# sdfgeoff/stereo_depth_estimation

Measured on AMD Instinct MI355X. Metric: stereo pairs/s training @320x240 bf16, 1/2/4/8 MI355X; EPE vs ref, higher is better.
Workload: dtype bf16

## Files before the change

stereo_depth_estimation_amd/csrc/bwd_fused.hip:

```cpp
#include <stdio.h>

#include "halo_util.h"

namespace {

typedef float f32x16 __attribute__((ext_vector_type(16)));

constexpr int FB_TH = 8, FB_TW = 16;
constexpr int FB_HW = FB_TW + 2, FB_HH = FB_TH + 2;
constexpr int FB_HPX = FB_HW * FB_HH;
constexpr int FB_NI = (FB_HPX * 4 + 255) / 256;
constexpr int FB_HSL = (FB_NI * 256 / 32) * 8;
static_assert(FB_TH * FB_TW == 128 && FB_TW % 16 == 0, "4 MFMA waves x 32 pixels; tr_pair rows p, p + 8 in one row");
constexpr int FB_DL = 40;
constexpr int FB_XL = 48;
constexpr int FB_XC = 64;
__device__ __forceinline__ int fb_xoff(int c) { return (c & 15) + (c >> 4) * FB_XC; }
constexpr int FB_WL = 9 * 32 + 8;
constexpr int FB_SL = 40;
constexpr int FB_DYH = FB_HSL * FB_DL, FB_XH = FB_HSL * FB_XL + (FB_XC - FB_XL + 16), FB_ST = FB_TH * FB_TW * FB_SL;
constexpr int FB_BUF = FB_DYH + FB_XH + FB_ST;
constexpr int FB_BLOCKS = 256;
#ifndef FB_EXP
#define FB_EXP 0
#endif
constexpr bool FB_DG = (FB_EXP & 32) != 0;
__device__ __forceinline__ unsigned long long fb_clk() {
    asm volatile("s_waitcnt lgkmcnt(0)" ::: "memory");
    return __builtin_amdgcn_s_memtime();
}

struct BwdArgs {
    const __bf16 *da, *y, *yp;
    const float *sc, *sh, *mu, *is, *coef;
    const float *psc, *psh, *pmu, *pis;
    const __bf16* wd;
    int kpad;
    int B, H, W, tiles_x, tiles_y;
    __bf16* dx;
    float* slab;
    float2* part;
    unsigned long long* dbg;
};

template <bool B> struct BoolC { static constexpr bool v = B; };

template <int PPX>
__device__ __forceinline__ int fb_pixel(int item) { return (item / (8 * PPX)) * 8 + (item & 7); }
template <int PPX>
__device__ __forceinline__ int fb_piece(int item) { return (item >> 3) % PPX; }

__device__ __forceinline__ void fb_tile(int tiles_x, int tiles_y, int bid, int nblk, int k, int& tx, int& ty, int& b) {
    const int strip = bid + (k / tiles_y) * nblk;
    ty = k % tiles_y;
    tx = strip % tiles_x;
    b = strip / tiles_x;
}
__device__ __forceinline__ int fb_ntile(int tiles_x, int tiles_y, int B, int bid, int nblk) {
    const int nstrips = tiles_x * B;
    return bid < nstrips ? ((nstrips - 1 - bid) / nblk + 1) * tiles_y : 0;
}

__global__ __launch_bounds__(512) void k_bwd_fused32(const BwdArgs p) {
    __shared__ __attribute__((aligned(16))) __bf16 smem[2 * FB_BUF];
    __shared__ __attribute__((aligned(16))) __bf16 wds[32 * FB_WL];
    __shared__ __attribute__((aligned(16))) __bf16 scr[4 * 32 * 32];
    __shared__ __attribute__((aligned(16))) float redf[4 * 32 * 2];

    const int tid = threadIdx.x, lane = tid & 63;
    const bool is_loader = tid >= 256;
    const int wid = (tid >> 6) & 3;
    const int bid = (blockIdx.x & 7) * (gridDim.x >> 3) + (blockIdx.x >> 3);
    const int t_begin = 0;
    const int ntile = fb_ntile(p.tiles_x, p.tiles_y, p.B, bid, gridDim.x);
    const int hw = p.H * p.W;

    for (int i = tid; i < 32 * 36; i += 512) {
        const int r = i / 36, c8 = i - r * 36;
        *reinterpret_cast<uint4*>(wds + r * FB_WL + c8 * 8) =
            *reinterpret_cast<const uint4*>(p.wd + (size_t)r * p.kpad + c8 * 8);
    }

    if (is_loader) {
        const int ltid = tid - 256;
        if (FB_EXP & 128) __builtin_amdgcn_s_setprio(1);
        const int piece = fb_piece<4>(ltid);
        constexpr unsigned OOB = 0x80000000u;
        float ksc[8], ksh[8], kB[8], kC[8];
#pragma unroll
        for (int j = 0; j < 8; ++j) {
            const int c = piece * 8 + j;
            const float k1 = p.coef[3 * c + 1], k2 = p.coef[3 * c + 2], is = p.is[c], sc = p.sc[c], sh = p.sh[c];
            ksc[j] = sc;
            ksh[j] = sh;
            kB[j] = -is * k2;
            kC[j] = is * k2 * sh + sc * (p.mu[c] * is * k2 - k1);
        }
        const float4 s0 = *reinterpret_cast<const float4*>(p.psc + piece * 8);
        const float4 s1 = *reinterpret_cast<const float4*>(p.psc + piece * 8 + 4);
        const float4 t0 = *reinterpret_cast<const float4*>(p.psh + piece * 8);
        const float4 t1 = *reinterpret_cast<const float4*>(p.psh + piece * 8 + 4);
        unsigned geo[FB_NI];
        int stash[FB_NI];
#pragma unroll
        for (int i = 0; i < FB_NI; ++i) {
            const int px = fb_pixel<4>(ltid + 256 * i);
            const int hy = px / FB_HW, hx = px - hy * FB_HW;
            geo[i] = px < FB_HPX ? (unsigned)(hy << 8 | hx) : 0xffffffffu;
            const bool in = px < FB_HPX && hy >= 1 && hy <= FB_TH && hx >= 1 && hx <= FB_TW;
            stash[i] = in ? ((hy - 1) * FB_TW + hx - 1) * FB_SL + piece * 8 : -1;
        }
        const bool w3 = (ltid & ~63) + 256 * (FB_NI - 1) < FB_HPX * 4;
        unsigned need = 0;
#pragma unroll
        for (int i = 0; i < FB_NI; ++i) need |= (unsigned)(geo[i] != 0xffffffffu) << i;
        struct Set {
            uint4 a[FB_NI], y[FB_NI], x[FB_NI];
            unsigned m;
            bool edge;
        };
        Set sa, sb;
        auto load = [&](Set& q, int tile) __attribute__((always_inline)) {
            if ((FB_EXP & 16) && tile >= t_begin + 2) return;
            const bool live = tile < t_begin + ntile;
            const int tl = live ? tile : t_begin;
            int tx, ty, b;
            fb_tile(p.tiles_x, p.tiles_y, bid, gridDim.x, tl, tx, ty, b);
            const int h0 = ty * FB_TH - 1, w0 = tx * FB_TW - 1;
            const size_t img = (size_t)b * hw * 32;
            const __amdgpu_buffer_rsrc_t ra =
                __builtin_amdgcn_make_buffer_rsrc((void*)(p.da + img), (short)0, hw * 64, 0x00020000);
            const __amdgpu_buffer_rsrc_t ry =
                __builtin_amdgcn_make_buffer_rsrc((void*)(p.y + img), (short)0, hw * 64, 0x00020000);
            const __amdgpu_buffer_rsrc_t rp =
                __builtin_amdgcn_make_buffer_rsrc((void*)(p.yp + img), (short)0, hw * 64, 0x00020000);
            unsigned m = 0;
#pragma unroll
            for (int i = 0; i < FB_NI; ++i) {
                if (i == FB_NI - 1 && !w3) break;
                const int h = h0 + (int)(geo[i] >> 8), w = w0 + (int)(geo[i] & 0xffu);
                const bool ok = live & (geo[i] != 0xffffffffu) & (h >= 0) & (h < p.H) & (w >= 0) & (w < p.W);
                m |= (unsigned)ok << i;
                const unsigned off = ok ? (unsigned)(h * p.W + w) * 64u + (unsigned)piece * 16u : OOB;
                const auto va = __builtin_amdgcn_raw_buffer_load_b128(ra, off, 0, 0);
                const auto vy = __builtin_amdgcn_raw_buffer_load_b128(ry, off, 0, 0);
                const auto vp = __builtin_amdgcn_raw_buffer_load_b128(rp, off, 0, 0);
                q.a[i] = make_uint4(va[0], va[1], va[2], va[3]);
                q.y[i] = make_uint4(vy[0], vy[1], vy[2], vy[3]);
                q.x[i] = make_uint4(vp[0], vp[1], vp[2], vp[3]);
            }
            q.m = m;
            q.edge = __builtin_amdgcn_ballot_w64(m != (w3 ? need : need & ((1u << (FB_NI - 1)) - 1))) != 0;
        };
        auto store = [&](Set& q, int buf) __attribute__((always_inline)) {
            __bf16* dyh = smem + buf * FB_BUF;
            __bf16* xh = dyh + FB_DYH;
            __bf16* st = xh + FB_XH;
            auto put = [&](auto SEL) __attribute__((always_inline)) {
#pragma unroll
                for (int i = 0; i < FB_NI; ++i) {
                    if (i == FB_NI - 1 && !w3) break;
                    const bool ok = (q.m >> i) & 1u;
                    const int px = fb_pixel<4>(ltid + 256 * i);
                    uint4 d = (FB_EXP & 1) ? q.a[i] : bn_bwd_pk(q.a[i], q.y[i], ksc, ksh, kB, kC);
                    uint4 x = (FB_EXP & 1) ? q.x[i] : bnrelu_pk(q.x[i], s0, s1, t0, t1);
                    if constexpr (decltype(SEL)::v) {
                        d = ok ? d : make_uint4(0, 0, 0, 0);
                        x = ok ? x : make_uint4(0, 0, 0, 0);
                    }
                    *reinterpret_cast<uint4*>(dyh + px * FB_DL + piece * 8) = d;
                    *reinterpret_cast<uint4*>(xh + px * FB_XL + fb_xoff(piece * 8)) = x;
                    if (stash[i] >= 0) *reinterpret_cast<uint4*>(st + stash[i]) = q.x[i];
                }
            };
            if (q.edge)
                put(BoolC<true>{});
            else
                put(BoolC<false>{});
        };
        load(sa, t_begin);
        __builtin_amdgcn_sched_barrier(0);
        load(sb, t_begin + 1);
        __syncthreads();
        unsigned long long tc[5] = {0, 0, 0, 0, 0}, tm0 = 0, t_all = FB_DG ? fb_clk() : 0;
        auto stamp = [&](int k) __attribute__((always_inline)) {
            if (FB_DG) {
                const unsigned long long t1 = fb_clk();
                tc[k] += t1 - tm0;
                tm0 = t1;
            }
        };
        for (int i = 0; i < ntile; i += 2) {
            if (FB_DG) {
                tm0 = fb_clk();
                asm volatile("s_waitcnt vmcnt(9)" ::: "memory");
                stamp(3);
            }
            store(sa, 0);
            stamp(0);
            load(sa, t_begin + i + 2);
            stamp(1);
            __syncthreads();
            stamp(2);
            if (FB_DG) {
                asm volatile("s_waitcnt vmcnt(9)" ::: "memory");
                stamp(3);
            }
            store(sb, 1);
            stamp(0);
            load(sb, t_begin + i + 3);
            stamp(1);
            __syncthreads();
            stamp(2);
        }
        if (FB_DG && p.dbg && lane == 0) {
            unsigned long long* d = p.dbg + ((size_t)bid * 8 + 4 + wid) * 8;
            d[0] = tc[0];
            d[1] = tc[1];
            d[2] = tc[2];
            d[3] = tc[3];
            d[4] = fb_clk() - t_all;
            d[5] = ntile;
        }
        __syncthreads();
        return;
    }

    __syncthreads();
    const int g = lane >> 4, q4 = (lane & 15) >> 2, pp = lane & 3;
    const int pk = 4 * (g >> 1) + q4, ch16 = 16 * (g & 1) + 4 * pp;
    const int tw0 = wid, tw1 = wid + 4;
    const int toffx0 = ((tw0 / 3) * FB_HW + tw0 % 3) * FB_XL, toffx1 = ((tw1 / 3) * FB_HW + tw1 % 3) * FB_XL;
    f32x16 accw[3];
#pragma unroll
    for (int t = 0; t < 3; ++t)
#pragma unroll
        for (int r = 0; r < 16; ++r) accw[t][r] = 0.f;
    BnsK bk[4];
    {
        const int c = (lane & 3) * 8;
#pragma unroll
        for (int q = 0; q < 4; ++q) {
            float v[4][2];
#pragma unroll
            for (int h = 0; h < 2; ++h) {
                const int ch = c + 2 * q + h;
                v[0][h] = p.psc[ch];
                v[1][h] = p.psh[ch];
                v[2][h] = p.pis[ch];
                v[3][h] = -p.pmu[ch] * p.pis[ch];
            }
            bk[q].sc = f32x2{v[0][0], v[0][1]};
            bk[q].sh = f32x2{v[1][0], v[1][1]};
            bk[q].is = f32x2{v[2][0], v[2][1]};
            bk[q].nmi = f32x2{v[3][0], v[3][1]};
        }
    }
    float own[16];
#pragma unroll
    for (int j = 0; j < 16; ++j) own[j] = 0.f;
    __bf16* const scw = scr + wid * 32 * 32;
    auto swz = [](int j, int px) { return j ^ ((px >> 1) & 3); };
    unsigned long long tc[6] = {0, 0, 0, 0, 0, 0}, t0 = 0, t_all = FB_DG ? fb_clk() : 0;
    auto stamp = [&](int k) __attribute__((always_inline)) {
        if (FB_DG) {
            const unsigned long long t1 = fb_clk();
            tc[k] += t1 - t0;
            t0 = t1;
        }
    };
    auto epilogue = [&](const f32x16& acc, const uint4* yv, int tl) __attribute__((always_inline)) {
        uint2 pk2[4];
#pragma unroll
        for (int g4 = 0; g4 < 4; ++g4) {
            bf16x4 v;
#pragma unroll
            for (int q = 0; q < 4; ++q) v[q] = (__bf16)acc[4 * g4 + q];
            pk2[g4] = *reinterpret_cast<uint2*>(&v);
        }
#pragma unroll
        for (int k = 0; k < 4; k += 2) {
            const auto rx = __builtin_amdgcn_permlane32_swap(pk2[k].x, pk2[k + 1].x, false, false);
            const auto ry = __builtin_amdgcn_permlane32_swap(pk2[k].y, pk2[k + 1].y, false, false);
            const int px = lane & 31, j = k + (lane >> 5);
            *reinterpret_cast<uint4*>(scw + px * 32 + swz(j, px) * 8) = make_uint4(rx[0], ry[0], rx[1], ry[1]);
        }
        asm volatile("" ::: "memory");
        int tx, ty, b;
        fb_tile(p.tiles_x, p.tiles_y, bid, gridDim.x, tl, tx, ty, b);
        const __amdgpu_buffer_rsrc_t rd = __builtin_amdgcn_make_buffer_rsrc(
            (void*)(p.dx + (size_t)b * hw * 32), (short)0, hw * 64, 0x00020000);
        uint4 vv[2];
#pragma unroll
        for (int rr = 0; rr < 2; ++rr) {
            const int px = rr * 16 + (lane >> 2), j = lane & 3;
            vv[rr] = *reinterpret_cast<const uint4*>(scw + px * 32 + swz(j, px) * 8);
        }
        asm volatile("" ::: "memory");
#pragma unroll
        for (int rr = 0; rr < 2; ++rr) {
            const int q = wid * 32 + rr * 16 + (lane >> 2), j = lane & 3;
            const int h = ty * FB_TH + q / FB_TW, w = tx * FB_TW + q % FB_TW;
            bns_add(own, vv[rr], yv[rr], true, bk);
            __attribute__((ext_vector_type(4))) unsigned data = {vv[rr].x, vv[rr].y, vv[rr].z, vv[rr].w};
            __builtin_amdgcn_raw_buffer_store_b128(data, rd, (unsigned)(h * p.W + w) * 64u + (unsigned)j * 16u, 0, 2);
        }
    };
    f32x16 accp;
    uint4 yvp[2];
    auto tile = [&](int it, auto EPI) __attribute__((always_inline)) {
        if (FB_DG) t0 = fb_clk();
        __syncthreads();
        stamp(0);
        const __bf16* dyh = smem + (it & 1) * FB_BUF;
        const __bf16* xh = dyh + FB_DYH;
        const __bf16* st = xh + FB_XH;
#pragma unroll
        for (int rr = 0; rr < FB_TH; ++rr) {
            const int r = (2 * wid + rr) & (FB_TH - 1);
            const __bf16* a0 = dyh + ((r + 1) * FB_HW + 1 + pk) * FB_DL + ch16;
            const bf16x8 af = tr_pair(a0, a0 + 8 * FB_DL);
            const __bf16* xr = xh + (r * FB_HW + pk) * FB_XL + fb_xoff(ch16);
            const bf16x8 b0 = tr_pair(xr + toffx0, xr + toffx0 + 8 * FB_XL);
            const bf16x8 b1 = tr_pair(xr + toffx1, xr + toffx1 + 8 * FB_XL);
            accw[0] = __builtin_amdgcn_mfma_f32_32x32x16_bf16(af, b0, accw[0], 0, 0, 0);
            accw[1] = __builtin_amdgcn_mfma_f32_32x32x16_bf16(af, b1, accw[1], 0, 0, 0);
            if (rr < 2) {
                const __bf16* x8 = xr + (2 * FB_HW + 2) * FB_XL;
                accw[2] = __builtin_amdgcn_mfma_f32_32x32x16_bf16(af, tr_pair(x8, x8 + 8 * FB_XL), accw[2], 0, 0, 0);
            }
            if constexpr (decltype(EPI)::v)
                if (rr == 2) epilogue(accp, yvp, t_begin + it - 1);
        }
        stamp(1);
        f32x16 accd;
#pragma unroll
        for (int r = 0; r < 16; ++r) accd[r] = 0.f;
        const int c8 = 8 * (lane >> 5);
        const __bf16* wrow = wds + (lane & 31) * FB_WL + c8;
        const int qd = wid * 32 + (lane & 31);
        const __bf16* drow = dyh + ((qd / FB_TW) * FB_HW + qd % FB_TW) * FB_DL + c8;
#pragma unroll
        for (int tap = 0; tap < 9; ++tap) {
            const int toff = ((tap / 3) * FB_HW + tap % 3) * FB_DL;
#pragma unroll
            for (int kk = 0; kk < 2; ++kk) {
                const bf16x8 a = *reinterpret_cast<const bf16x8*>(wrow + tap * 32 + kk * 16);
                const bf16x8 b = *reinterpret_cast<const bf16x8*>(drow + toff + kk * 16);
                accd = __builtin_amdgcn_mfma_f32_32x32x16_bf16(a, b, accd, 0, 0, 0);
            }
        }
        accp = accd;
#pragma unroll
        for (int rr = 0; rr < 2; ++rr) {
            const int px = rr * 16 + (lane >> 2), j = lane & 3;
            yvp[rr] = *reinterpret_cast<const uint4*>(st + (wid * 32 + px) * FB_SL + j * 8);
        }
        stamp(2);
    };
    if (ntile > 0) tile(0, BoolC<false>{});
    for (int it = 1; it < ntile; ++it) tile(it, BoolC<true>{});
    if (ntile > 0) epilogue(accp, yvp, t_begin + ntile - 1);
    if (FB_DG && p.dbg && lane == 0) {
        unsigned long long* d = p.dbg + ((size_t)bid * 8 + wid) * 8;
#pragma unroll
        for (int k = 0; k < 6; ++k) d[k] = tc[k];
        d[6] = fb_clk() - t_all;
        d[7] = ntile;
    }
    if (ntile & 1) __syncthreads();

    float* slab = p.slab + (size_t)bid * 32 * 288;
    float* red8 = reinterpret_cast<float*>(smem + (ntile & 1) * FB_BUF);
    static_assert(FB_BUF * 2 >= 4 * 1024 * 4, "tap-8 partials fit one halo buffer");
#pragma unroll
    for (int i = 0; i < 16; ++i) {
        const int co = 8 * (i / 4) + 4 * (lane >> 5) + i % 4, ci = lane & 31;
        slab[(size_t)co * 288 + tw0 * 32 + ci] = accw[0][i];
        slab[(size_t)co * 288 + tw1 * 32 + ci] = accw[1][i];
        red8[wid * 1024 + co * 32 + ci] = accw[2][i];
    }
#pragma unroll
    for (int k = 0; k < 16; ++k)
#pragma unroll
        for (int o = 4; o < 64; o <<= 1) own[k] += __shfl_xor(own[k], o);
    if (lane < 4) {
#pragma unroll
        for (int k = 0; k < 16; ++k)
            redf[(wid * 32 + lane * 8 + k / 2) * 2 + (k & 1)] = own[(k & ~3) | ((k & 1) << 1) | ((k >> 1) & 1)];
    }
    __syncthreads();
#pragma unroll
    for (int e = tid; e < 1024; e += 256)
        slab[(size_t)(e >> 5) * 288 + 8 * 32 + (e & 31)] = (red8[e] + red8[1024 + e]) + (red8[2048 + e] + red8[3072 + e]);
    if (tid < 32) {
        float s = 0.f, sx = 0.f;
#pragma unroll
        for (int w = 0; w < 4; ++w) {
            s += redf[(w * 32 + tid) * 2];
            sx += redf[(w * 32 + tid) * 2 + 1];
        }
        p.part[(size_t)bid * 32 + tid] = make_float2(s, sx);
    }
}


struct DecArgs {
    const __bf16 *da, *y, *xu, *xs;
    const float *sc, *sh, *mu, *is, *coef;
    const float *ssc, *ssh;
    const __bf16* wd;
    int kpad;
    int B, H, W, tiles_x, tiles_y;
    __bf16 *du, *dsk;
    float* slab;
    float2* part;
    unsigned long long* dbg;
};
constexpr int FD_BUF = FB_DYH + 2 * FB_XH;

__global__ __launch_bounds__(512) void k_bwd_fused_dec(const DecArgs p) {
    __shared__ __attribute__((aligned(16))) __bf16 smem[2 * FD_BUF];
    __shared__ __attribute__((aligned(16))) __bf16 wds[64 * FB_WL];
    __shared__ __attribute__((aligned(16))) __bf16 scr[4 * 32 * 32];
    __shared__ __attribute__((aligned(16))) float redf[4 * 32];

    const int tid = threadIdx.x, lane = tid & 63;
    const bool is_loader = tid >= 256;
    const int wid = (tid >> 6) & 3;
    const int bid = (blockIdx.x & 7) * (gridDim.x >> 3) + (blockIdx.x >> 3);
    const int t_begin = 0;
    const int ntile = fb_ntile(p.tiles_x, p.tiles_y, p.B, bid, gridDim.x);
    const int hw = p.H * p.W;
    auto tile_of = [&](int tl, int& tx, int& ty, int& b) __attribute__((always_inline)) {
        fb_tile(p.tiles_x, p.tiles_y, bid, gridDim.x, tl, tx, ty, b);
    };

    for (int i = tid; i < 64 * 36; i += 512) {
        const int r = i / 36, c8 = i - r * 36;
        *reinterpret_cast<uint4*>(wds + r * FB_WL + c8 * 8) =
            *reinterpret_cast<const uint4*>(p.wd + (size_t)r * p.kpad + c8 * 8);
    }

    if (is_loader) {
        const int ltid = tid - 256;
        const int piece = fb_piece<4>(ltid);
        constexpr unsigned OOB = 0x80000000u;
        float ksc[8], ksh[8], kB[8], kC[8];
#pragma unroll
        for (int j = 0; j < 8; ++j) {
            const int c = piece * 8 + j;
            const float k1 = p.coef[3 * c + 1], k2 = p.coef[3 * c + 2], is = p.is[c], sc = p.sc[c], sh = p.sh[c];
            ksc[j] = sc;
            ksh[j] = sh;
            kB[j] = -is * k2;
            kC[j] = is * k2 * sh + sc * (p.mu[c] * is * k2 - k1);
        }
        const float4 s0 = *reinterpret_cast<const float4*>(p.ssc + piece * 8);
        const float4 s1 = *reinterpret_cast<const float4*>(p.ssc + piece * 8 + 4);
        const float4 t0 = *reinterpret_cast<const float4*>(p.ssh + piece * 8);
        const float4 t1 = *reinterpret_cast<const float4*>(p.ssh + piece * 8 + 4);
        unsigned geo[FB_NI];
#pragma unroll
        for (int i = 0; i < FB_NI; ++i) {
            const int px = fb_pixel<4>(ltid + 256 * i);
            const int hy = px / FB_HW, hx = px - hy * FB_HW;
            geo[i] = px < FB_HPX ? (unsigned)(hy << 8 | hx) : 0xffffffffu;
        }
        const bool w3 = (ltid & ~63) + 256 * (FB_NI - 1) < FB_HPX * 4;
        unsigned need = 0;
#pragma unroll
        for (int i = 0; i < FB_NI; ++i) need |= (unsigned)(geo[i] != 0xffffffffu) << i;
        struct Set {
            uint4 a[FB_NI], y[FB_NI], u[FB_NI], s[FB_NI];
            unsigned m;
            bool edge;
        };
        Set sa, sb;
        auto load = [&](Set& q, int tile) __attribute__((always_inline)) {
            const bool live = tile < t_begin + ntile;
            int tx, ty, b;
            tile_of(live ? tile : t_begin, tx, ty, b);
            const int h0 = ty * FB_TH - 1, w0 = tx * FB_TW - 1;
            const size_t img = (size_t)b * hw * 32;
            const __amdgpu_buffer_rsrc_t ra =
                __builtin_amdgcn_make_buffer_rsrc((void*)(p.da + img), (short)0, hw * 64, 0x00020000);
            const __amdgpu_buffer_rsrc_t ry =
                __builtin_amdgcn_make_buffer_rsrc((void*)(p.y + img), (short)0, hw * 64, 0x00020000);
            const __amdgpu_buffer_rsrc_t ru =
                __builtin_amdgcn_make_buffer_rsrc((void*)(p.xu + img), (short)0, hw * 64, 0x00020000);
            const __amdgpu_buffer_rsrc_t rs =
                __builtin_amdgcn_make_buffer_rsrc((void*)(p.xs + img), (short)0, hw * 64, 0x00020000);
            unsigned m = 0;
#pragma unroll
            for (int i = 0; i < FB_NI; ++i) {
                if (i == FB_NI - 1 && !w3) break;
                const int h = h0 + (int)(geo[i] >> 8), w = w0 + (int)(geo[i] & 0xffu);
                const bool ok = live & (geo[i] != 0xffffffffu) & (h >= 0) & (h < p.H) & (w >= 0) & (w < p.W);
                m |= (unsigned)ok << i;
                const unsigned off = ok ? (unsigned)(h * p.W + w) * 64u + (unsigned)piece * 16u : OOB;
                const auto va = __builtin_amdgcn_raw_buffer_load_b128(ra, off, 0, 0);
                const auto vy = __builtin_amdgcn_raw_buffer_load_b128(ry, off, 0, 0);
                const auto vu = __builtin_amdgcn_raw_buffer_load_b128(ru, off, 0, 0);
                const auto vs = __builtin_amdgcn_raw_buffer_load_b128(rs, off, 0, 0);
                q.a[i] = make_uint4(va[0], va[1], va[2], va[3]);
                q.y[i] = make_uint4(vy[0], vy[1], vy[2], vy[3]);
                q.u[i] = make_uint4(vu[0], vu[1], vu[2], vu[3]);
                q.s[i] = make_uint4(vs[0], vs[1], vs[2], vs[3]);
            }
            q.m = m;
            q.edge = __builtin_amdgcn_ballot_w64(m != (w3 ? need : need & ((1u << (FB_NI - 1)) - 1))) != 0;
        };
        auto store = [&](Set& q, int buf) __attribute__((always_inline)) {
            __bf16* dyh = smem + buf * FD_BUF;
            __bf16* xuh = dyh + FB_DYH;
            __bf16* xsh = xuh + FB_XH;
            auto put = [&](auto SEL) __attribute__((always_inline)) {
#pragma unroll
                for (int i = 0; i < FB_NI; ++i) {
                    if (i == FB_NI - 1 && !w3) break;
                    const bool ok = (q.m >> i) & 1u;
                    const int px = fb_pixel<4>(ltid + 256 * i);
                    uint4 d = bn_bwd_pk(q.a[i], q.y[i], ksc, ksh, kB, kC);
                    uint4 xs = bnrelu_pk(q.s[i], s0, s1, t0, t1);
                    uint4 xu = q.u[i];
                    if constexpr (decltype(SEL)::v) {
                        d = ok ? d : make_uint4(0, 0, 0, 0);
                        xs = ok ? xs : make_uint4(0, 0, 0, 0);
                        xu = ok ? xu : make_uint4(0, 0, 0, 0);
                    }
                    *reinterpret_cast<uint4*>(dyh + px * FB_DL + piece * 8) = d;
                    *reinterpret_cast<uint4*>(xuh + px * FB_XL + fb_xoff(piece * 8)) = xu;
                    *reinterpret_cast<uint4*>(xsh + px * FB_XL + fb_xoff(piece * 8)) = xs;
                }
            };
            if (q.edge)
                put(BoolC<true>{});
            else
                put(BoolC<false>{});
        };
        load(sa, t_begin);
        __builtin_amdgcn_sched_barrier(0);
        load(sb, t_begin + 1);
        __syncthreads();
        unsigned long long tc[3] = {0, 0, 0}, tm0 = 0, t_all = FB_DG ? fb_clk() : 0;
        auto stamp = [&](int k) __attribute__((always_inline)) {
            if (FB_DG) {
                const unsigned long long t1 = fb_clk();
                tc[k] += t1 - tm0;
                tm0 = t1;
            }
        };
        for (int i = 0; i < ntile; i += 2) {
            if (FB_DG) tm0 = fb_clk();
            store(sa, 0);
            stamp(0);
            load(sa, t_begin + i + 2);
            stamp(1);
            __syncthreads();
            stamp(2);
            store(sb, 1);
            stamp(0);
            load(sb, t_begin + i + 3);
            stamp(1);
            __syncthreads();
            stamp(2);
        }
        if (FB_DG && p.dbg && lane == 0) {
            unsigned long long* d = p.dbg + ((size_t)bid * 8 + 4 + wid) * 8;
            d[0] = tc[0];
            d[1] = tc[1];
            d[2] = tc[2];
            d[3] = 0;
            d[4] = fb_clk() - t_all;
            d[5] = ntile;
        }
        __syncthreads();
        return;
    }

    __syncthreads();
    const int g = lane >> 4, q4 = (lane & 15) >> 2, pp = lane & 3;
    const int pk = 4 * (g >> 1) + q4, ch16 = 16 * (g & 1) + 4 * pp;
    const int hh = wid & 1, tg = wid >> 1;
    int toffx[4];
#pragma unroll
    for (int j = 0; j < 4; ++j) {
        const int t = 4 * tg + j;
        toffx[j] = ((t / 3) * FB_HW + t % 3) * FB_XL;
    }
    f32x16 accw[5];
#pragma unroll
    for (int t = 0; t < 5; ++t)
#pragma unroll
        for (int r = 0; r < 16; ++r) accw[t][r] = 0.f;
    float ownb[8];
#pragma unroll
    for (int j = 0; j < 8; ++j) ownb[j] = 0.f;
    __bf16* const scw = scr + wid * 32 * 32;
    auto swz = [](int j, int px) { return j ^ ((px >> 1) & 3); };
    auto epilogue = [&](const f32x16& acc, __bf16* out, bool bias, int tl) __attribute__((always_inline)) {
        uint2 pk2[4];
#pragma unroll
        for (int g4 = 0; g4 < 4; ++g4) {
            bf16x4 v;
#pragma unroll
            for (int q = 0; q < 4; ++q) v[q] = (__bf16)acc[4 * g4 + q];
            pk2[g4] = *reinterpret_cast<uint2*>(&v);
        }
#pragma unroll
        for (int k = 0; k < 4; k += 2) {
            const auto rx = __builtin_amdgcn_permlane32_swap(pk2[k].x, pk2[k + 1].x, false, false);
            const auto ry = __builtin_amdgcn_permlane32_swap(pk2[k].y, pk2[k + 1].y, false, false);
            const int px = lane & 31, j = k + (lane >> 5);
            *reinterpret_cast<uint4*>(scw + px * 32 + swz(j, px) * 8) = make_uint4(rx[0], ry[0], rx[1], ry[1]);
        }
        asm volatile("" ::: "memory");
        int tx, ty, b;
        tile_of(tl, tx, ty, b);
        const __amdgpu_buffer_rsrc_t rd =
            __builtin_amdgcn_make_buffer_rsrc((void*)(out + (size_t)b * hw * 32), (short)0, hw * 64, 0x00020000);
        uint4 vv[2];
#pragma unroll
        for (int rr = 0; rr < 2; ++rr) {
            const int px = rr * 16 + (lane >> 2), j = lane & 3;
            vv[rr] = *reinterpret_cast<const uint4*>(scw + px * 32 + swz(j, px) * 8);
        }
        asm volatile("" ::: "memory");
#pragma unroll
        for (int rr = 0; rr < 2; ++rr) {
            const int q = wid * 32 + rr * 16 + (lane >> 2), j = lane & 3;
            const int h = ty * FB_TH + q / FB_TW, w = tx * FB_TW + q % FB_TW;
            if (bias) {
                const unsigned wv[4] = {vv[rr].x, vv[rr].y, vv[rr].z, vv[rr].w};
#pragma unroll
                for (int e = 0; e < 4; ++e) {
                    ownb[2 * e] += __uint_as_float(wv[e] << 16);
                    ownb[2 * e + 1] += __uint_as_float(wv[e] & 0xffff0000u);
                }
            }
            __attribute__((ext_vector_type(4))) unsigned data = {vv[rr].x, vv[rr].y, vv[rr].z, vv[rr].w};
            __builtin_amdgcn_raw_buffer_store_b128(data, rd, (unsigned)(h * p.W + w) * 64u + (unsigned)j * 16u, 0, 2);
        }
    };
    unsigned long long tc[4] = {0, 0, 0, 0}, t0 = 0, t_all = FB_DG ? fb_clk() : 0;
    auto stamp = [&](int k) __attribute__((always_inline)) {
        if (FB_DG) {
            const unsigned long long t1 = fb_clk();
            tc[k] += t1 - t0;
            t0 = t1;
        }
    };
    f32x16 accp0, accp1;
    auto tile = [&](int it, auto EPI) __attribute__((always_inline)) {
        if (FB_DG) t0 = fb_clk();
        __syncthreads();
        stamp(0);
        const __bf16* dyh = smem + (it & 1) * FD_BUF;
        const __bf16* xsrc = dyh + FB_DYH + hh * FB_XH;
#pragma unroll
        for (int rr = 0; rr < FB_TH; ++rr) {
            const int r = (4 * tg + rr) & (FB_TH - 1);
            const __bf16* a0 = dyh + ((r + 1) * FB_HW + 1 + pk) * FB_DL + ch16;
            const bf16x8 af = tr_pair(a0, a0 + 8 * FB_DL);
            const __bf16* xr = xsrc + (r * FB_HW + pk) * FB_XL + fb_xoff(ch16);
#pragma unroll
            for (int j = 0; j < 4; ++j) {
                const bf16x8 bfr = tr_pair(xr + toffx[j], xr + toffx[j] + 8 * FB_XL);
                accw[j] = __builtin_amdgcn_mfma_f32_32x32x16_bf16(af, bfr, accw[j], 0, 0, 0);
            }
            if (rr < 4) {
                const __bf16* x8 = xr + (2 * FB_HW + 2) * FB_XL;
                accw[4] = __builtin_amdgcn_mfma_f32_32x32x16_bf16(af, tr_pair(x8, x8 + 8 * FB_XL), accw[4], 0, 0, 0);
            }
            if constexpr (decltype(EPI)::v) {
                if (rr == 1) epilogue(accp0, p.du, true, t_begin + it - 1);
                if (rr == 5) epilogue(accp1, p.dsk, false, t_begin + it - 1);
            }
        }
        stamp(1);
        f32x16 accd0, accd1;
#pragma unroll
        for (int r = 0; r < 16; ++r) accd0[r] = accd1[r] = 0.f;
        const int c8 = 8 * (lane >> 5);
        const __bf16* wrow = wds + (lane & 31) * FB_WL + c8;
        const int qd = wid * 32 + (lane & 31);
        const __bf16* drow = dyh + ((qd / FB_TW) * FB_HW + qd % FB_TW) * FB_DL + c8;
#pragma unroll
        for (int tap = 0; tap < 9; ++tap) {
            const int toff = ((tap / 3) * FB_HW + tap % 3) * FB_DL;
#pragma unroll
            for (int kk = 0; kk < 2; ++kk) {
                const bf16x8 bdy = *reinterpret_cast<const bf16x8*>(drow + toff + kk * 16);
                const bf16x8 a0 = *reinterpret_cast<const bf16x8*>(wrow + tap * 32 + kk * 16);
                const bf16x8 a1 = *reinterpret_cast<const bf16x8*>(wrow + 32 * FB_WL + tap * 32 + kk * 16);
                accd0 = __builtin_amdgcn_mfma_f32_32x32x16_bf16(a0, bdy, accd0, 0, 0, 0);
                accd1 = __builtin_amdgcn_mfma_f32_32x32x16_bf16(a1, bdy, accd1, 0, 0, 0);
            }
        }
        accp0 = accd0;
        accp1 = accd1;
        stamp(2);
    };
    if (ntile > 0) tile(0, BoolC<false>{});
    for (int it = 1; it < ntile; ++it) tile(it, BoolC<true>{});
    if (FB_DG && p.dbg && lane == 0) {
        unsigned long long* d = p.dbg + ((size_t)bid * 8 + wid) * 8;
#pragma unroll
        for (int k = 0; k < 4; ++k) d[k] = tc[k];
        d[4] = d[5] = 0;
        d[6] = fb_clk() - t_all;
        d[7] = ntile;
    }
    if (ntile > 0) {
        epilogue(accp0, p.du, true, t_begin + ntile - 1);
        epilogue(accp1, p.dsk, false, t_begin + ntile - 1);
    }
    if (ntile & 1) __syncthreads();

    float* slab = p.slab + (size_t)bid * 32 * 576;
    float* red8 = reinterpret_cast<float*>(smem + (ntile & 1) * FD_BUF);
    static_assert(FD_BUF * 2 >= 4 * 1024 * 4, "tap-8 partials fit one halo buffer");
#pragma unroll
    for (int i = 0; i < 16; ++i) {
        const int co = 8 * (i / 4) + 4 * (lane >> 5) + i % 4, ci = hh * 32 + (lane & 31);
#pragma unroll
        for (int j = 0; j < 4; ++j) slab[(size_t)co * 576 + (4 * tg + j) * 64 + ci] = accw[j][i];
        red8[wid * 1024 + co * 32 + (lane & 31)] = accw[4][i];
    }
#pragma unroll
    for (int k = 0; k < 8; ++k)
#pragma unroll
        for (int o = 4; o < 64; o <<= 1) ownb[k] += __shfl_xor(ownb[k], o);
    if (lane < 4) {
#pragma unroll
        for (int k = 0; k < 8; ++k) redf[wid * 32 + lane * 8 + k] = ownb[k];
    }
    __syncthreads();
    for (int e = tid; e < 2 * 1024; e += 256) {
        const int h2 = e >> 10, r = e & 1023;
        slab[(size_t)(r >> 5) * 576 + 8 * 64 + h2 * 32 + (r & 31)] = red8[h2 * 1024 + r] + red8[(h2 + 2) * 1024 + r];
    }
    if (tid < 32)
        p.part[(size_t)bid * 32 + tid] =
            make_float2((redf[tid] + redf[32 + tid]) + (redf[64 + tid] + redf[96 + tid]), 0.f);
}

}

unsigned long long* sd_debug_ptr();

extern "C" int sd_conv3x3_bwd_fused_ok(int C, int Cx, int H, int W) {
    return C == 32 && Cx == 32 && H % FB_TH == 0 && W % FB_TW == 0 && W / FB_TW < 256 && (long long)H * W * 64 < (1LL << 31)
               ? 1
               : 0;
}

extern "C" int sd_conv3x3_bwd_fused_splits(int batch, int H, int W) {
    const long long ns = (long long)batch * (W / FB_TW);
    return ns < FB_BLOCKS ? (int)((ns + 7) / 8 * 8) : FB_BLOCKS;
}

extern "C" int sd_conv3x3_bwd_fused(const void* da, const void* y, const float* scale, const float* shift,
                                    const float* mean, const float* invstd, const float* coef, const void* yp,
                                    const float* pscale, const float* pshift, const float* pmean, const float* pinvstd,
                                    const void* wd, int kpad, int batch, int H, int W, void* dx, float* slab,
                                    float* partials, sd_stream s) {
    SD_REQUIRE(sd_conv3x3_bwd_fused_ok(32, 32, H, W) == 1 && batch > 0,
               "sd_conv3x3_bwd_fused: 32 -> 32 channels, H %% %d == 0, W %% %d == 0 (got %dx%d)", FB_TH, FB_TW, H, W);
    SD_REQUIRE(da && y && scale && shift && mean && invstd && coef && yp && pscale && pshift && pmean && pinvstd && wd &&
                   dx && slab && partials && kpad >= 288,
               "sd_conv3x3_bwd_fused: bad args");
    BwdArgs p;
    p.da = (const __bf16*)da;
    p.y = (const __bf16*)y;
    p.yp = (const __bf16*)yp;
    p.sc = scale;
    p.sh = shift;
    p.mu = mean;
    p.is = invstd;
    p.coef = coef;
    p.psc = pscale;
    p.psh = pshift;
    p.pmu = pmean;
    p.pis = pinvstd;
    p.wd = (const __bf16*)wd;
    p.kpad = kpad;
    p.B = batch;
    p.H = H;
    p.W = W;
    p.tiles_x = W / FB_TW;
    p.tiles_y = H / FB_TH;
    const long long nt = (long long)batch * p.tiles_x * p.tiles_y;
    SD_REQUIRE(nt < (1LL << 30), "sd_conv3x3_bwd_fused: too many tiles");
    const int blocks = sd_conv3x3_bwd_fused_splits(batch, H, W);
    p.dx = (__bf16*)dx;
    p.slab = slab;
    p.part = reinterpret_cast<float2*>(partials);
    p.dbg = FB_DG ? sd_debug_ptr() : nullptr;
    hipLaunchKernelGGL(k_bwd_fused32, dim3(blocks), dim3(512), 0, to_stream(s), p);
    return sd_check_launch("sd_conv3x3_bwd_fused");
}

extern "C" int sd_conv3x3_bwd_fused_dec_ok(int C, int Cu, int Cs, int H, int W) {
    return C == 32 && Cu == 32 && Cs == 32 && sd_conv3x3_bwd_fused_ok(32, 32, H, W) == 1 ? 1 : 0;
}

extern "C" int sd_conv3x3_bwd_fused_dec(const void* da, const void* y, const float* scale, const float* shift,
                                        const float* mean, const float* invstd, const float* coef, const void* xu,
                                        const void* xs, const float* sscale, const float* sshift, const void* wd,
                                        int kpad, int batch, int H, int W, void* du, void* dskip, float* slab,
                                        float* partials, sd_stream s) {
    SD_REQUIRE(sd_conv3x3_bwd_fused_dec_ok(32, 32, 32, H, W) == 1 && batch > 0,
               "sd_conv3x3_bwd_fused_dec: 32 + 32 -> 32 channels, H %% %d == 0, W %% %d == 0 (got %dx%d)", FB_TH,
               FB_TW, H, W);
    SD_REQUIRE(da && y && scale && shift && mean && invstd && coef && xu && xs && sscale && sshift && wd && du &&
                   dskip && slab && partials && kpad >= 288,
               "sd_conv3x3_bwd_fused_dec: bad args");
    DecArgs p;
    p.da = (const __bf16*)da;
    p.y = (const __bf16*)y;
    p.xu = (const __bf16*)xu;
    p.xs = (const __bf16*)xs;
    p.sc = scale;
    p.sh = shift;
    p.mu = mean;
    p.is = invstd;
    p.coef = coef;
    p.ssc = sscale;
    p.ssh = sshift;
    p.wd = (const __bf16*)wd;
    p.kpad = kpad;
    p.B = batch;
    p.H = H;
    p.W = W;
    p.tiles_x = W / FB_TW;
    p.tiles_y = H / FB_TH;
    const long long nt = (long long)batch * p.tiles_x * p.tiles_y;
    SD_REQUIRE(nt < (1LL << 30), "sd_conv3x3_bwd_fused_dec: too many tiles");
    const int blocks = sd_conv3x3_bwd_fused_splits(batch, H, W);
    p.du = (__bf16*)du;
    p.dsk = (__bf16*)dskip;
    p.slab = slab;
    p.part = reinterpret_cast<float2*>(partials);
    p.dbg = FB_DG ? sd_debug_ptr() : nullptr;
    hipLaunchKernelGGL(k_bwd_fused_dec, dim3(blocks), dim3(512), 0, to_stream(s), p);
    return sd_check_launch("sd_conv3x3_bwd_fused_dec");
}
```

Baseline: 7513.

## Carry halo rows between vertically adjacent tiles in fused conv backward kernels

Each block walks a column strip top to bottom. The change reuses the overlapping halo rows of the previous tile's shared-memory buffers (dy and x) instead of reloading them from global memory. The loaders are rearranged into body and head items so the carried rows are skipped, and a fast path for interior tiles drops the per-pixel bounds checks. This adds LDS copies and more complex index bookkeeping, and the stash region grows by one row. The behaviour can be turned off with an environment variable.

After: 7525, median of 6. About the same (+0.2%).

```diff
diff --git a/stereo_depth_estimation_amd/csrc/bwd_fused.hip b/stereo_depth_estimation_amd/csrc/bwd_fused.hip
--- a/stereo_depth_estimation_amd/csrc/bwd_fused.hip
+++ b/stereo_depth_estimation_amd/csrc/bwd_fused.hip
@@ -1,16 +1,23 @@
 #include <stdio.h>
+#include <stdlib.h>
 
 #include "halo_util.h"
 
 namespace {
 
 typedef float f32x16 __attribute__((ext_vector_type(16)));
+typedef unsigned u32x4 __attribute__((ext_vector_type(4)));
 
 constexpr int FB_TH = 8, FB_TW = 16;
 constexpr int FB_HW = FB_TW + 2, FB_HH = FB_TH + 2;
 constexpr int FB_HPX = FB_HW * FB_HH;
 constexpr int FB_NI = (FB_HPX * 4 + 255) / 256;
 constexpr int FB_HSL = (FB_NI * 256 / 32) * 8;
+constexpr int FB_HEAD = 2 * FB_HW;
+constexpr int FB_NBODY = (FB_HPX - FB_HEAD) / 16;
+static_assert(FB_NI == 3 && FB_NBODY == 9 && FB_NBODY * 16 == FB_HPX - FB_HEAD && FB_HEAD <= 48 &&
+                  FB_HPX + 48 - FB_HEAD <= FB_HSL,
+              "fb_item: 9 body + 3 head wave-items per kind over 4 waves x 3 slots; head lanes past row 1 in spare slots");
 static_assert(FB_TH * FB_TW == 128 && FB_TW % 16 == 0, "4 MFMA waves x 32 pixels; tr_pair rows p, p + 8 in one row");
 constexpr int FB_DL = 40;
 constexpr int FB_XL = 48;
@@ -18,7 +25,7 @@
 __device__ __forceinline__ int fb_xoff(int c) { return (c & 15) + (c >> 4) * FB_XC; }
 constexpr int FB_WL = 9 * 32 + 8;
 constexpr int FB_SL = 40;
-constexpr int FB_DYH = FB_HSL * FB_DL, FB_XH = FB_HSL * FB_XL + (FB_XC - FB_XL + 16), FB_ST = FB_TH * FB_TW * FB_SL;
+constexpr int FB_DYH = FB_HSL * FB_DL, FB_XH = FB_HSL * FB_XL + (FB_XC - FB_XL + 16), FB_ST = (FB_TH + 1) * FB_TW * FB_SL;
 constexpr int FB_BUF = FB_DYH + FB_XH + FB_ST;
 constexpr int FB_BLOCKS = 256;
 #ifndef FB_EXP
@@ -40,6 +47,7 @@
     __bf16* dx;
     float* slab;
     float2* part;
+    int carry;
     unsigned long long* dbg;
 };
 
@@ -60,6 +68,54 @@
     const int nstrips = tiles_x * B;
     return bid < nstrips ? ((nstrips - 1 - bid) / nblk + 1) * tiles_y : 0;
 }
+
+struct FbWalk {
+    int tx, ty, b, strip;
+    __device__ __forceinline__ FbWalk(int tiles_x, int bid) : tx(bid % tiles_x), ty(0), b(bid / tiles_x), strip(bid) {}
+    __device__ __forceinline__ void next(int tiles_x, int tiles_y, int nblk) {
+        if (++ty == tiles_y) {
+            ty = 0;
+            strip += nblk;
+            tx = strip % tiles_x;
+            b = strip / tiles_x;
+        }
+    }
+};
+
+__device__ __forceinline__ bool fb_item(bool xkind, int lw, int i, int lp, unsigned& geo, int& slot) {
+    const bool head = xkind ? lw == 0 : lw != 0 && i == FB_NI - 1;
+    const int n = xkind ? (head ? i : 3 * lw - 3 + i) : (head ? lw - 1 : (lw == 0 ? i : 2 * lw + 1 + i));
+    const int px = (head ? 0 : FB_HEAD) + 16 * n + lp;
+    const bool valid = !head || px < FB_HEAD;
+    geo = valid ? (unsigned)((px / FB_HW) << 8 | (px % FB_HW)) : 0xffffffffu;
+    slot = valid ? px : FB_HPX + px - FB_HEAD;
+    return head;
+}
+template <int NX, bool STASH>
+__device__ __forceinline__ bool fb_copy(int c, int& src, int& dst) {
+    constexpr int NH = FB_HEAD * 4;
+    const int pc = c & 3;
+    if (c < NH) {
+        dst = (c >> 2) * FB_DL + pc * 8;
+        src = dst + FB_TH * FB_HW * FB_DL;
+        return true;
+    }
+    if (c < NH * (1 + NX)) {
+        const int a = (c - NH) / NH, r = (c - NH) % NH;
+        dst = FB_DYH + a * FB_XH + (r >> 2) * FB_XL + fb_xoff(pc * 8);
+        src = dst + FB_TH * FB_HW * FB_XL;
+        return true;
+    }
+    if (STASH && c < NH * (1 + NX) + FB_TW * 4) {
+        dst = FB_DYH + NX * FB_XH + ((c - NH * (1 + NX)) >> 2) * FB_SL + pc * 8;
+        src = dst + FB_TH * FB_TW * FB_SL;
+        return true;
+    }
+    src = dst = (FB_HSL - 1) * FB_DL;
+    return false;
+}
+template <int NX, bool STASH>
+constexpr int FB_NCP = (FB_HEAD * 4 * (1 + NX) + (STASH ? FB_TW * 4 : 0) + 255) / 256;
 
 __global__ __launch_bounds__(512) void k_bwd_fused32(const BwdArgs p) {
     __shared__ __attribute__((aligned(16))) __bf16 smem[2 * FB_BUF];
@@ -100,32 +156,46 @@
         const float4 s1 = *reinterpret_cast<const float4*>(p.psc + piece * 8 + 4);
         const float4 t0 = *reinterpret_cast<const float4*>(p.psh + piece * 8);
         const float4 t1 = *reinterpret_cast<const float4*>(p.psh + piece * 8 + 4);
-        unsigned geo[FB_NI];
-        int stash[FB_NI];
+        const int lw = __builtin_amdgcn_readfirstlane(ltid >> 6), lp = (lane >> 5) * 8 + (lane & 7);
+        const bool head_d = lw != 0, head_x = lw == 0;
+        unsigned gd[FB_NI], gx[FB_NI], need = 0, need_body = 0;
+        int od[FB_NI], ox[FB_NI], stash[FB_NI];
+        unsigned vd[FB_NI], vx[FB_NI];
 #pragma unroll
         for (int i = 0; i < FB_NI; ++i) {
-            const int px = fb_pixel<4>(ltid + 256 * i);
-            const int hy = px / FB_HW, hx = px - hy * FB_HW;
-            geo[i] = px < FB_HPX ? (unsigned)(hy << 8 | hx) : 0xffffffffu;
-            const bool in = px < FB_HPX && hy >= 1 && hy <= FB_TH && hx >= 1 && hx <= FB_TW;
-            stash[i] = in ? ((hy - 1) * FB_TW + hx - 1) * FB_SL + piece * 8 : -1;
-        }
-        const bool w3 = (ltid & ~63) + 256 * (FB_NI - 1) < FB_HPX * 4;
-        unsigned need = 0;
-#pragma unroll
-        for (int i = 0; i < FB_NI; ++i) need |= (unsigned)(geo[i] != 0xffffffffu) << i;
+            int sd, sx;
+            const bool hd = fb_item(false, lw, i, lp, gd[i], sd), hx = fb_item(true, lw, i, lp, gx[i], sx);
+            od[i] = sd * FB_DL + piece * 8;
+            ox[i] = sx * FB_XL + fb_xoff(piece * 8);
+            const bool hasd = gd[i] != 0xffffffffu, hasx = gx[i] != 0xffffffffu;
+            need |= (unsigned)hasd << i | (unsigned)hasx << (FB_NI + i);
+            need_body |= (unsigned)(hasd && !hd) << i | (unsigned)(hasx && !hx) << (FB_NI + i);
+            vd[i] = hasd ? ((gd[i] >> 8) * (unsigned)p.W + (gd[i] & 0xffu)) * 64u + (unsigned)piece * 16u : OOB;
+            vx[i] = hasx ? ((gx[i] >> 8) * (unsigned)p.W + (gx[i] & 0xffu)) * 64u + (unsigned)piece * 16u : OOB;
+            const int ry = (int)(gx[i] >> 8), rx = (int)(gx[i] & 0xffu);
+            const bool in = gx[i] != 0xffffffffu && ry >= 1 && ry <= FB_TH + 1 && rx >= 1 && rx <= FB_TW;
+            stash[i] = in ? ((ry - 1) * FB_TW + rx - 1) * FB_SL + piece * 8 : -1;
+        }
+        constexpr int NCP = FB_NCP<1, true>;
+        static_assert(NCP == 2, "store's cp0, cp1");
+        int csrc[NCP], cdst[NCP];
+#pragma unroll
+        for (int j = 0; j < NCP; ++j) fb_copy<1, true>(ltid + 256 * j, csrc[j], cdst[j]);
         struct Set {
             uint4 a[FB_NI], y[FB_NI], x[FB_NI];
             unsigned m;
             bool edge;
+            bool carry;
         };
         Set sa, sb;
+        FbWalk walk(p.tiles_x, bid);
         auto load = [&](Set& q, int tile) __attribute__((always_inline)) {
+            const bool live = tile < t_begin + ntile;
+            const int tx = live ? walk.tx : 0, ty = live ? walk.ty : 0, b = live ? walk.b : 0;
+            walk.next(p.tiles_x, p.tiles_y, gridDim.x);
+            const bool carry = live && ty > 0 && p.carry != 0;
             if ((FB_EXP & 16) && tile >= t_begin + 2) return;
-            const bool live = tile < t_begin + ntile;
-            const int tl = live ? tile : t_begin;
-            int tx, ty, b;
-            fb_tile(p.tiles_x, p.tiles_y, bid, gridDim.x, tl, tx, ty, b);
+            q.carry = carry;
             const int h0 = ty * FB_TH - 1, w0 = tx * FB_TW - 1;
             const size_t img = (size_t)b * hw * 32;
             const __amdgpu_buffer_rsrc_t ra =
@@ -134,55 +204,87 @@
                 __builtin_amdgcn_make_buffer_rsrc((void*)(p.y + img), (short)0, hw * 64, 0x00020000);
             const __amdgpu_buffer_rsrc_t rp =
                 __builtin_amdgcn_make_buffer_rsrc((void*)(p.yp + img), (short)0, hw * 64, 0x00020000);
-            unsigned m = 0;
+            const bool skd = carry && head_d, skx = carry && head_x;
+            const bool inner = live && ty > 0 && ty + 1 < p.tiles_y && tx > 0 && tx + 1 < p.tiles_x;
+            const unsigned base = (unsigned)(h0 * p.W + w0) * 64u;
+            unsigned offd[FB_NI], offx[FB_NI], m = carry ? need_body : need;
+            if (inner) {
+#pragma unroll
+                for (int i = 0; i < FB_NI; ++i) {
+                    offd[i] = skd && i == FB_NI - 1 ? OOB : vd[i] + base;
+                    offx[i] = skx ? OOB : vx[i] + base;
+                }
+                q.edge = false;
+            } else {
+                m = 0;
+#pragma unroll
+                for (int i = 0; i < FB_NI; ++i) {
+                    const int hd = h0 + (int)(gd[i] >> 8), wd = w0 + (int)(gd[i] & 0xffu);
+                    const int hx = h0 + (int)(gx[i] >> 8), wx = w0 + (int)(gx[i] & 0xffu);
+                    const bool okd = live & !(skd && i == FB_NI - 1) & (gd[i] != 0xffffffffu) & (hd >= 0) & (hd < p.H) &
+                                     (wd >= 0) & (wd < p.W);
+                    const bool okx =
+                        live & !skx & (gx[i] != 0xffffffffu) & (hx >= 0) & (hx < p.H) & (wx >= 0) & (wx < p.W);
+                    m |= (unsigned)okd << i | (unsigned)okx << (FB_NI + i);
+                    offd[i] = okd ? vd[i] + base : OOB;
+                    offx[i] = okx ? vx[i] + base : OOB;
+                }
+                q.edge = __builtin_amdgcn_ballot_w64(m != (carry ? need_body : need)) != 0;
+            }
+            q.m = m;
 #pragma unroll
             for (int i = 0; i < FB_NI; ++i) {
-                if (i == FB_NI - 1 && !w3) break;
-                const int h = h0 + (int)(geo[i] >> 8), w = w0 + (int)(geo[i] & 0xffu);
-                const bool ok = live & (geo[i] != 0xffffffffu) & (h >= 0) & (h < p.H) & (w >= 0) & (w < p.W);
-                m |= (unsigned)ok << i;
-                const unsigned off = ok ? (unsigned)(h * p.W + w) * 64u + (unsigned)piece * 16u : OOB;
-                const auto va = __builtin_amdgcn_raw_buffer_load_b128(ra, off, 0, 0);
-                const auto vy = __builtin_amdgcn_raw_buffer_load_b128(ry, off, 0, 0);
-                const auto vp = __builtin_amdgcn_raw_buffer_load_b128(rp, off, 0, 0);
+                const auto va = __builtin_amdgcn_raw_buffer_load_b128(ra, offd[i], 0, 0);
+                const auto vy = __builtin_amdgcn_raw_buffer_load_b128(ry, offd[i], 0, 0);
+                const auto vp = __builtin_amdgcn_raw_buffer_load_b128(rp, offx[i], 0, 0);
                 q.a[i] = make_uint4(va[0], va[1], va[2], va[3]);
                 q.y[i] = make_uint4(vy[0], vy[1], vy[2], vy[3]);
                 q.x[i] = make_uint4(vp[0], vp[1], vp[2], vp[3]);
             }
-            q.m = m;
-            q.edge = __builtin_amdgcn_ballot_w64(m != (w3 ? need : need & ((1u << (FB_NI - 1)) - 1))) != 0;
         };
         auto store = [&](Set& q, int buf) __attribute__((always_inline)) {
             __bf16* dyh = smem + buf * FB_BUF;
             __bf16* xh = dyh + FB_DYH;
             __bf16* st = xh + FB_XH;
+            u32x4 cp0, cp1;
+            if (q.carry) {
+                const __bf16* prev = smem + (buf ^ 1) * FB_BUF;
+                cp0 = *reinterpret_cast<const u32x4*>(prev + csrc[0]);
+                cp1 = *reinterpret_cast<const u32x4*>(prev + csrc[1]);
+            }
+            const bool skd = q.carry && head_d, skx = q.carry && head_x;
             auto put = [&](auto SEL) __attribute__((always_inline)) {
 #pragma unroll
                 for (int i = 0; i < FB_NI; ++i) {
-                    if (i == FB_NI - 1 && !w3) break;
-                    const bool ok = (q.m >> i) & 1u;
-                    const int px = fb_pixel<4>(ltid + 256 * i);
-                    uint4 d = (FB_EXP & 1) ? q.a[i] : bn_bwd_pk(q.a[i], q.y[i], ksc, ksh, kB, kC);
-                    uint4 x = (FB_EXP & 1) ? q.x[i] : bnrelu_pk(q.x[i], s0, s1, t0, t1);
-                    if constexpr (decltype(SEL)::v) {
-                        d = ok ? d : make_uint4(0, 0, 0, 0);
-                        x = ok ? x : make_uint4(0, 0, 0, 0);
+                    if (!(skd && i == FB_NI - 1)) {
+                        uint4 d = (FB_EXP & 1) ? q.a[i] : bn_bwd_pk(q.a[i], q.y[i], ksc, ksh, kB, kC);
+                        if constexpr (decltype(SEL)::v)
+                            d = (q.m >> i) & 1u ? d : make_uint4(0, 0, 0, 0);
+                        *reinterpret_cast<uint4*>(dyh + od[i]) = d;
                     }
-                    *reinterpret_cast<uint4*>(dyh + px * FB_DL + piece * 8) = d;
-                    *reinterpret_cast<uint4*>(xh + px * FB_XL + fb_xoff(piece * 8)) = x;
-                    if (stash[i] >= 0) *reinterpret_cast<uint4*>(st + stash[i]) = q.x[i];
+                    if (!skx) {
+                        uint4 x = (FB_EXP & 1) ? q.x[i] : bnrelu_pk(q.x[i], s0, s1, t0, t1);
+                        if constexpr (decltype(SEL)::v) x = (q.m >> (FB_NI + i)) & 1u ? x : make_uint4(0, 0, 0, 0);
+                        *reinterpret_cast<uint4*>(xh + ox[i]) = x;
+                        if (stash[i] >= 0) *reinterpret_cast<uint4*>(st + stash[i]) = q.x[i];
+                    }
                 }
             };
             if (q.edge)
                 put(BoolC<true>{});
             else
                 put(BoolC<false>{});
+            if (q.carry) {
+                *reinterpret_cast<u32x4*>(dyh + cdst[0]) = cp0;
+                *reinterpret_cast<u32x4*>(dyh + cdst[1]) = cp1;
+            }
         };
         load(sa, t_begin);
         __builtin_amdgcn_sched_barrier(0);
         load(sb, t_begin + 1);
         __syncthreads();
         unsigned long long tc[5] = {0, 0, 0, 0, 0}, tm0 = 0, t_all = FB_DG ? fb_clk() : 0;
+        const unsigned long long r_all = FB_DG ? __builtin_amdgcn_s_memrealtime() : 0;
         auto stamp = [&](int k) __attribute__((always_inline)) {
             if (FB_DG) {
                 const unsigned long long t1 = fb_clk();
@@ -221,6 +323,7 @@
             d[3] = tc[3];
             d[4] = fb_clk() - t_all;
             d[5] = ntile;
+            d[6] = __builtin_amdgcn_s_memrealtime() - r_all;
         }
         __syncthreads();
         return;
@@ -415,6 +518,7 @@
     __bf16 *du, *dsk;
     float* slab;
     float2* part;
+    int carry;
     unsigned long long* dbg;
 };
 constexpr int FD_BUF = FB_DYH + 2 * FB_XH;
@@ -460,27 +564,41 @@
         const float4 s1 = *reinterpret_cast<const float4*>(p.ssc + piece * 8 + 4);
         const float4 t0 = *reinterpret_cast<const float4*>(p.ssh + piece * 8);
         const float4 t1 = *reinterpret_cast<const float4*>(p.ssh + piece * 8 + 4);
-        unsigned geo[FB_NI];
+        const int lw = __builtin_amdgcn_readfirstlane(ltid >> 6), lp = (lane >> 5) * 8 + (lane & 7);
+        const bool head_d = lw != 0, head_x = lw == 0;
+        unsigned gd[FB_NI], gx[FB_NI], need = 0, need_body = 0;
+        int od[FB_NI], ox[FB_NI];
+        unsigned vd[FB_NI], vx[FB_NI];
 #pragma unroll
         for (int i = 0; i < FB_NI; ++i) {
-            const int px = fb_pixel<4>(ltid + 256 * i);
-            const int hy = px / FB_HW, hx = px - hy * FB_HW;
-            geo[i] = px < FB_HPX ? (unsigned)(hy << 8 | hx) : 0xffffffffu;
-        }
-        const bool w3 = (ltid & ~63) + 256 * (FB_NI - 1) < FB_HPX * 4;
-        unsigned need = 0;
-#pragma unroll
-        for (int i = 0; i < FB_NI; ++i) need |= (unsigned)(geo[i] != 0xffffffffu) << i;
+            int sd, sx;
+            const bool hd = fb_item(false, lw, i, lp, gd[i], sd), hx = fb_item(true, lw, i, lp, gx[i], sx);
+            od[i] = sd * FB_DL + piece * 8;
+            ox[i] = sx * FB_XL + fb_xoff(piece * 8);
+            const bool hasd = gd[i] != 0xffffffffu, hasx = gx[i] != 0xffffffffu;
+            need |= (unsigned)hasd << i | (unsigned)hasx << (FB_NI + i);
+            need_body |= (unsigned)(hasd && !hd) << i | (unsigned)(hasx && !hx) << (FB_NI + i);
+            vd[i] = hasd ? ((gd[i] >> 8) * (unsigned)p.W + (gd[i] & 0xffu)) * 64u + (unsigned)piece * 16u : OOB;
+            vx[i] = hasx ? ((gx[i] >> 8) * (unsigned)p.W + (gx[i] & 0xffu)) * 64u + (unsigned)piece * 16u : OOB;
+        }
+        constexpr int NCP = FB_NCP<2, false>;
+        static_assert(NCP == 2, "store's cp0, cp1");
+        int csrc[NCP], cdst[NCP];
+#pragma unroll
+        for (int j = 0; j < NCP; ++j) fb_copy<2, false>(ltid + 256 * j, csrc[j], cdst[j]);
         struct Set {
             uint4 a[FB_NI], y[FB_NI], u[FB_NI], s[FB_NI];
             unsigned m;
-            bool edge;
+            bool edge, carry;
         };
         Set sa, sb;
+        FbWalk walk(p.tiles_x, bid);
         auto load = [&](Set& q, int tile) __attribute__((always_inline)) {
             const bool live = tile < t_begin + ntile;
-            int tx, ty, b;
-            tile_of(live ? tile : t_begin, tx, ty, b);
+            const int tx = live ? walk.tx : 0, ty = live ? walk.ty : 0, b = live ? walk.b : 0;
+            walk.next(p.tiles_x, p.tiles_y, gridDim.x);
+            const bool carry = live && ty > 0 && p.carry != 0;
+            q.carry = carry;
             const int h0 = ty * FB_TH - 1, w0 = tx * FB_TW - 1;
             const size_t img = (size_t)b * hw * 32;
             const __amdgpu_buffer_rsrc_t ra =
@@ -491,59 +609,94 @@
                 __builtin_amdgcn_make_buffer_rsrc((void*)(p.xu + img), (short)0, hw * 64, 0x00020000);
             const __amdgpu_buffer_rsrc_t rs =
                 __builtin_amdgcn_make_buffer_rsrc((void*)(p.xs + img), (short)0, hw * 64, 0x00020000);
-            unsigned m = 0;
+            const bool skd = carry && head_d, skx = carry && head_x;
+            const bool inner = live && ty > 0 && ty + 1 < p.tiles_y && tx > 0 && tx + 1 < p.tiles_x;
+            const unsigned base = (unsigned)(h0 * p.W + w0) * 64u;
+            unsigned offd[FB_NI], offx[FB_NI], m = carry ? need_body : need;
+            if (inner) {
+#pragma unroll
+                for (int i = 0; i < FB_NI; ++i) {
+                    offd[i] = skd && i == FB_NI - 1 ? OOB : vd[i] + base;
+                    offx[i] = skx ? OOB : vx[i] + base;
+                }
+                q.edge = false;
+            } else {
+                m = 0;
+#pragma unroll
+                for (int i = 0; i < FB_NI; ++i) {
+                    const int hd = h0 + (int)(gd[i] >> 8), wd = w0 + (int)(gd[i] & 0xffu);
+                    const int hx = h0 + (int)(gx[i] >> 8), wx = w0 + (int)(gx[i] & 0xffu);
+                    const bool okd = live & !(skd && i == FB_NI - 1) & (gd[i] != 0xffffffffu) & (hd >= 0) & (hd < p.H) &
+                                     (wd >= 0) & (wd < p.W);
+                    const bool okx =
+                        live & !skx & (gx[i] != 0xffffffffu) & (hx >= 0) & (hx < p.H) & (wx >= 0) & (wx < p.W);
+                    m |= (unsigned)okd << i | (unsigned)okx << (FB_NI + i);
+                    offd[i] = okd ? vd[i] + base : OOB;
+                    offx[i] = okx ? vx[i] + base : OOB;
+                }
+                q.edge = __builtin_amdgcn_ballot_w64(m != (carry ? need_body : need)) != 0;
+            }
+            q.m = m;
 #pragma unroll
             for (int i = 0; i < FB_NI; ++i) {
-                if (i == FB_NI - 1 && !w3) break;
-                const int h = h0 + (int)(geo[i] >> 8), w = w0 + (int)(geo[i] & 0xffu);
-                const bool ok = live & (geo[i] != 0xffffffffu) & (h >= 0) & (h < p.H) & (w >= 0) & (w < p.W);
-                m |= (unsigned)ok << i;
-                const unsigned off = ok ? (unsigned)(h * p.W + w) * 64u + (unsigned)piece * 16u : OOB;
-                const auto va = __builtin_amdgcn_raw_buffer_load_b128(ra, off, 0, 0);
-                const auto vy = __builtin_amdgcn_raw_buffer_load_b128(ry, off, 0, 0);
-                const auto vu = __builtin_amdgcn_raw_buffer_load_b128(ru, off, 0, 0);
-                const auto vs = __builtin_amdgcn_raw_buffer_load_b128(rs, off, 0, 0);
+                const auto va = __builtin_amdgcn_raw_buffer_load_b128(ra, offd[i], 0, 0);
+                const auto vy = __builtin_amdgcn_raw_buffer_load_b128(ry, offd[i], 0, 0);
+                const auto vu = __builtin_amdgcn_raw_buffer_load_b128(ru, offx[i], 0, 0);
+                const auto vs = __builtin_amdgcn_raw_buffer_load_b128(rs, offx[i], 0, 0);
                 q.a[i] = make_uint4(va[0], va[1], va[2], va[3]);
                 q.y[i] = make_uint4(vy[0], vy[1], vy[2], vy[3]);
                 q.u[i] = make_uint4(vu[0], vu[1], vu[2], vu[3]);
                 q.s[i] = make_uint4(vs[0], vs[1], vs[2], vs[3]);
             }
-            q.m = m;
-            q.edge = __builtin_amdgcn_ballot_w64(m != (w3 ? need : need & ((1u << (FB_NI - 1)) - 1))) != 0;
         };
         auto store = [&](Set& q, int buf) __attribute__((always_inline)) {
             __bf16* dyh = smem + buf * FD_BUF;
             __bf16* xuh = dyh + FB_DYH;
             __bf16* xsh = xuh + FB_XH;
+            u32x4 cp0, cp1;
+            if (q.carry) {
+                const __bf16* prev = smem + (buf ^ 1) * FD_BUF;
+                cp0 = *reinterpret_cast<const u32x4*>(prev + csrc[0]);
+                cp1 = *reinterpret_cast<const u32x4*>(prev + csrc[1]);
+            }
+            const bool skd = q.carry && head_d, skx = q.carry && head_x;
             auto put = [&](auto SEL) __attribute__((always_inline)) {
 #pragma unroll
                 for (int i = 0; i < FB_NI; ++i) {
-                    if (i == FB_NI - 1 && !w3) break;
-                    const bool ok = (q.m >> i) & 1u;
-                    const int px = fb_pixel<4>(ltid + 256 * i);
-                    uint4 d = bn_bwd_pk(q.a[i], q.y[i], ksc, ksh, kB, kC);
-                    uint4 xs = bnrelu_pk(q.s[i], s0, s1, t0, t1);
-                    uint4 xu = q.u[i];
-                    if constexpr (decltype(SEL)::v) {
-                        d = ok ? d : make_uint4(0, 0, 0, 0);
-                        xs = ok ? xs : make_uint4(0, 0, 0, 0);
-                        xu = ok ? xu : make_uint4(0, 0, 0, 0);
+                    if (!(skd && i == FB_NI - 1)) {
+                        uint4 d = bn_bwd_pk(q.a[i], q.y[i], ksc, ksh, kB, kC);
+                        if constexpr (decltype(SEL)::v)
+                            d = (q.m >> i) & 1u ? d : make_uint4(0, 0, 0, 0);
+                        *reinterpret_cast<uint4*>(dyh + od[i]) = d;
                     }
-                    *reinterpret_cast<uint4*>(dyh + px * FB_DL + piece * 8) = d;
-                    *reinterpret_cast<uint4*>(xuh + px * FB_XL + fb_xoff(piece * 8)) = xu;
-                    *reinterpret_cast<uint4*>(xsh + px * FB_XL + fb_xoff(piece * 8)) = xs;
+                    if (!skx) {
+                        uint4 xs = bnrelu_pk(q.s[i], s0, s1, t0, t1);
+                        uint4 xu = q.u[i];
+                        if constexpr (decltype(SEL)::v) {
+                            const bool ok = (q.m >> (FB_NI + i)) & 1u;
+                            xs = ok ? xs : make_uint4(0, 0, 0, 0);
+                            xu = ok ? xu : make_uint4(0, 0, 0, 0);
+                        }
+                        *reinterpret_cast<uint4*>(xuh + ox[i]) = xu;
+                        *reinterpret_cast<uint4*>(xsh + ox[i]) = xs;
+                    }
                 }
             };
             if (q.edge)
                 put(BoolC<true>{});
             else
                 put(BoolC<false>{});
+            if (q.carry) {
+                *reinterpret_cast<u32x4*>(dyh + cdst[0]) = cp0;
+                *reinterpret_cast<u32x4*>(dyh + cdst[1]) = cp1;
+            }
         };
         load(sa, t_begin);
         __builtin_amdgcn_sched_barrier(0);
         load(sb, t_begin + 1);
         __syncthreads();
         unsigned long long tc[3] = {0, 0, 0}, tm0 = 0, t_all = FB_DG ? fb_clk() : 0;
+        const unsigned long long r_all = FB_DG ? __builtin_amdgcn_s_memrealtime() : 0;
         auto stamp = [&](int k) __attribute__((always_inline)) {
             if (FB_DG) {
                 const unsigned long long t1 = fb_clk();
@@ -574,6 +727,7 @@
             d[3] = 0;
             d[4] = fb_clk() - t_all;
             d[5] = ntile;
+            d[6] = __builtin_amdgcn_s_memrealtime() - r_all;
         }
         __syncthreads();
         return;
@@ -749,6 +903,11 @@
 }
 
 unsigned long long* sd_debug_ptr();
+
+static int bwd_carry_enabled() {
+    const char* e = getenv("SD_BWD_CARRY");
+    return !(e && *e && atoi(e) == 0);
+}
 
 extern "C" int sd_conv3x3_bwd_fused_ok(int C, int Cx, int H, int W) {
     return C == 32 && Cx == 32 && H % FB_TH == 0 && W % FB_TW == 0 && W / FB_TW < 256 && (long long)H * W * 64 < (1LL << 31)
@@ -797,6 +956,7 @@
     p.dx = (__bf16*)dx;
     p.slab = slab;
     p.part = reinterpret_cast<float2*>(partials);
+    p.carry = bwd_carry_enabled();
     p.dbg = FB_DG ? sd_debug_ptr() : nullptr;
     hipLaunchKernelGGL(k_bwd_fused32, dim3(blocks), dim3(512), 0, to_stream(s), p);
     return sd_check_launch("sd_conv3x3_bwd_fused");
@@ -843,6 +1003,7 @@
     p.dsk = (__bf16*)dskip;
     p.slab = slab;
     p.part = reinterpret_cast<float2*>(partials);
+    p.carry = bwd_carry_enabled();
     p.dbg = FB_DG ? sd_debug_ptr() : nullptr;
     hipLaunchKernelGGL(k_bwd_fused_dec, dim3(blocks), dim3(512), 0, to_stream(s), p);
     return sd_check_launch("sd_conv3x3_bwd_fused_dec");
```
